# wheretrue/exon-duckdb

Measured on AMD Instinct MI355X. Metric: FASTQ records/sec into DataChunks, higher is better.
Workload: dtype u8; 1 GPU; read_fastq on 10 GB synthetic 150 bp FASTQ (332 B/record, 30120481 records), 1x MI355X, byte-range shards; bytes_per_gpu=9999999692, columns=name,description,sequence,quality_scores as duckdb::string_t + validity

## Files before the change

### exon_duckdb_amd/arrow.py

```python
import ctypes as C

from ._lib import ExgError, load_library
from . import abi


class ReaderResult(C.Structure):
    _fields_ = [("error", C.c_void_p)]


_bound = False


def _lib():
    global _bound
    l = load_library()
    if not _bound:
        l.new_reader.restype = ReaderResult
        l.new_reader.argtypes = [C.c_void_p, C.c_char_p, C.c_size_t, C.c_char_p, C.c_char_p, C.c_char_p]
        _bound = True
    return l


def new_reader(uri, file_format, batch_size=abi.EXG_VECTOR_SIZE, compression=None, filters=None):
    import pyarrow as pa

    l = _lib()
    stream = (C.c_uint64 * 8)()
    enc = lambda s: None if s is None else s.encode()
    res = l.new_reader(C.addressof(stream), enc(uri), batch_size, enc(compression), enc(file_format), enc(filters))
    if res.error:
        msg = C.string_at(res.error).decode("utf-8", "replace")
        C.CDLL(None).free(C.c_void_p(res.error))
        raise ExgError(abi.EXG_E_INVALID_ARG, msg)
    return pa.RecordBatchReader._import_from_c(C.addressof(stream))
```

### exon_duckdb_amd/csrc/exg_fastq_fused.hip

```cpp
#include "exg_fastq.hpp"
#include "exg_fused_core.hpp"

namespace exg {

struct FastqFormat;
static constexpr int kFastqHalves = 3;


__device__ __forceinline__ void fastq_report_utf8(ScanWsHeader *hdr, long long out, int64_t rec_off) {
    atomicMin(&hdr->err_word, ((unsigned long long)out << 8) | EXG_PE_INVALID_UTF8);
    atomicMin(&hdr->err_off, (unsigned long long)rec_off);
}

template <int kMode, class L>
__device__ __forceinline__ void fastq_emit_half(const L &s, const FastqDev &a, ScanWsHeader *hdr, const TileCtx &c,
                                          unsigned long long halo_nl, uint32_t dev_mode, uint32_t lane,
                                          uint32_t wave, unsigned long long *__restrict__ tile_qend,
                                          uint64_t tile_index) {
    const unsigned long long P0 = a.first_line_index - halo_nl;
    const uint32_t i0 = (uint32_t)((3 - P0) & 3);
    const uint32_t i_first = (uint32_t)((3 - (P0 + c.P)) & 3);
    const unsigned long long q_before = c.P > i0 ? (c.P - i0 + 3) / 4 : 0;
    const unsigned long long n_hc = halo_nl > i0 ? (halo_nl - i0 + 3) / 4 : 0;
    const uint32_t n_rec = c.n_lines > i_first ? (c.n_lines - i_first + 3) / 4 : 0;
    const uint64_t ptr_of_e0 = a.payload_base + c.tile_off - kWin;

    if (threadIdx.x == 0 && (c.pass_base == 0 || n_rec)) {
        long long e = 0;
        if (n_rec) {
            e = (long long)c.tile_off + (int)s.nlist[4 + i_first + 4 * (n_rec - 1)] - kWin + 1;
            if ((unsigned long long)e > a.n_bytes) e = (long long)a.n_bytes;
        }
        if (c.pass_base) e |= (long long)(tile_qend[tile_index] & kFarBit);
        if constexpr (kMode != kLean) if (n_rec && s.nlist[i_first] == kNoneE) {
            const long long out0 = (long long)q_before - (long long)n_hc;
            const int e4 = s.nlist[4 + i_first];
            if ((uint64_t)((int64_t)c.tile_off + e4 - kWin) >= a.lead && out0 >= 0 &&
                ((a.flags & EXG_F_NO_STORE) || (unsigned long long)out0 < a.capacity)) {
                FarRec f;
#pragma unroll
                for (int k = 0; k < 5; k++) {
                    const uint32_t idx = i_first + k;
                    f.pos[k] = idx >= 4 ? c.half * kTile + (int32_t)s.nlist[idx] - kWin : s.prev32[idx];
                }
                f.flags = c.is_eof_tile ? 1u : 0u;
                f.out = out0;
                far_rec_of(tile_qend, a.n_bytes)[tile_index] = f;
                hdr->any_far = 1u;
                e |= (long long)kFarBit;
            }
        }
        tile_qend[tile_index] = (unsigned long long)e;
    }
    if (dev_mode >= 3) return;
    const bool no_store = (a.flags & EXG_F_NO_STORE) != 0;

    for (uint32_t jb = 0; jb < n_rec; jb += 64) {
        const uint32_t j = jb + lane;
        const long long out = (long long)(q_before + j) - (long long)n_hc;
        bool act = j < n_rec;
        int i = 0;
        if (act) {
            i = (int)(i_first + 4 * j);
            int e4 = s.nlist[4 + i];
            act = (uint64_t)((int64_t)c.tile_off + e4 - kWin) >= a.lead && out >= 0;
            if (act && !no_store && (unsigned long long)out >= a.capacity) {
                if (wave == 0) atomicOr(&hdr->flags, EXG_RF_CAPACITY);
                act = false;
            }
        }
        bool desc_valid = false;
        if (act) {
            const uint32_t q0 = s.nlist[i];
            uint4 val = make_uint4(0, 0, 0, 0);
            if (q0 == kNoneE) {
                if constexpr (kMode == kLean) {
                    if (wave == 0) {
                        tile_redo_of(tile_qend, a.n_bytes)[opaque_s((uint32_t)(tile_index / kFastqHalves))] = kRedoFar;
                        hdr->any_redo = 1u;
                    }
                }
            } else if (wave <= 1) {
                int s0 = (int)q0 + 1, e0 = s.nlist[i + 1];
                bool name_ok = s0 < e0 && ldb(s, s0) == '@';
                if (e0 > s0 && !(c.is_eof_tile && e0 == c.lim_e) && ldb(s, e0 - 1) == '\r') e0--;
                int ns = s0 + 1 < e0 ? s0 + 1 : e0;
                int sp = e0;
                for (uint32_t aa = (uint32_t)ns & ~3u; aa < (uint32_t)e0 && sp == e0; aa += 32) {
                    uint32_t w8[8];
#pragma unroll
                    for (int q = 0; q < 8; q++) w8[q] = ldw(s, aa + 4 * q);
                    uint32_t bits = 0;
#pragma unroll
                    for (int q = 0; q < 8; q++) bits |= nib4(match4(w8[q], 0x20202020u)) << (4 * q);
                    if (aa < (uint32_t)ns) bits &= 0xFFFFFFFFu << ((uint32_t)ns - aa);
                    if (bits) {
                        uint32_t pos = aa + (uint32_t)__ffs(bits) - 1;
                        if (pos < (uint32_t)e0) sp = (int)pos;
                        break;
                    }
                }
                int ds = sp < e0 ? sp + 1 : e0;
// ... 198 lines not shown
    r.flags = hdr->flags | (hdr->any_redo ? EXG_RF_REDO : 0u);
    r.payload_bytes = 0;
    r.redo_tiles = hdr->n_redo;
    r.error_code = 0;
    r.error_offset = ~0ull;
    r.error_record = ~0ull;
    uint64_t n_rec = (n_owned < a.capacity || (a.flags & EXG_F_NO_STORE)) ? n_owned : a.capacity;
    if (err != kNoError) {
        uint64_t rec = err >> 8;
        r.error_code = (uint32_t)(err & 0xFF);
        r.error_record = rec;
        r.error_offset = err_off;
        if (rec < n_rec) {
            n_rec = rec;
            consumed = err_off > a.lead ? err_off : a.lead;
        }
    }
    r.n_records = n_rec;
    r.consumed_bytes = n_rec ? consumed : a.lead;
    *res = r;
}

int run_fastq_fused(const exg_fastq_scan_args *args, const FastqDev &dev_in, uint8_t *ws, const FastqWsLayout &l,
                    hipStream_t stream, bool full) {
    FastqDev dev = dev_in;
#ifdef EXG_DEV_PROBE
    if (const char *e = getenv("EXG_FASTQ_DEV_MODE")) dev.flags |= ((uint32_t)atoi(e) & 31u) << 8;
#endif
    ScanWsHeader *hdr = reinterpret_cast<ScanWsHeader *>(ws);
    constexpr uint64_t kSuperBytes = (uint64_t)FastqFormat::kHalves * kTile;
    constexpr uint32_t kHalvesHost = FastqFormat::kHalves;
    uint64_t n_super64 = (dev.n_bytes + kSuperBytes - 1) / kSuperBytes;
    if (n_super64 == 0) n_super64 = 1;
    if (n_super64 > 0x7FFFFFF0ull) {
        set_error("exg_fastq_scan: buffer too large for one launch (%llu super-tiles)", (unsigned long long)n_super64);
        return EXG_E_INVALID_ARG;
    }
    uint32_t n_super = (uint32_t)n_super64;
    const uint64_t n = l.n_tiles_fused;
    unsigned int *tileA = reinterpret_cast<unsigned int *>(ws + l.off_tile_desc);
    unsigned long long *tileP = reinterpret_cast<unsigned long long *>(ws + l.off_tile_desc) + n;
    unsigned long long *tile_qend = tileP + 2 * n;
    int32_t *tileL = reinterpret_cast<int32_t *>(ws + l.off_tile_last4);
    FarRec *far_rec = reinterpret_cast<FarRec *>(ws + l.off_far);
    hipLaunchKernelGGL(k_init_hdr, dim3(1), dim3(1), 0, stream, hdr, l.lines_cap, 0u);
    EXG_HIP_CHECK(hipMemsetAsync(tileA, 0, (size_t)n * 24, stream));
    if (dev.lead) {
        int rc = exg_count_newlines(dev.d_in, 0, dev.lead, (uint64_t *)&hdr->halo_nl, stream);
        if (rc) return rc;
    }
    if (full) {
        hipLaunchKernelGGL((k_fused<FastqFormat, kFullPrimary>), dim3(n_super + 1), dim3(kThreads), 0, stream, dev, tileA, tileP, tile_qend, hdr, n_super);
    } else {
        hipLaunchKernelGGL((k_fused<FastqFormat, kLean>), dim3(n_super + 1), dim3(kThreads), 0, stream, dev, tileA, tileP, tile_qend, hdr, n_super);
        hipLaunchKernelGGL((k_fused<FastqFormat, kFullRedo>), dim3(n_super < 1280 ? n_super : 1280), dim3(kThreads), 0, stream, dev, tileA, tileP,
                           tile_qend, hdr, n_super);
    }
    {
        const uint32_t n_halves = n_super * kHalvesHost;
        const uint32_t grid = (n_halves + 255) / 256 < 4096 ? (n_halves + 255) / 256 : 4096;
        hipLaunchKernelGGL(k_fastq_far, dim3(grid), dim3(256), 0, stream, dev, tileA, tileL, tile_qend, far_rec, hdr, n_halves);
    }
    hipLaunchKernelGGL(k_fastq_finalize_fused, dim3(1), dim3(256), 0, stream, dev, hdr, tile_qend, n_super * kHalvesHost,
                       args->d_result);
    EXG_HIP_CHECK(hipGetLastError());
    return EXG_OK;
}

}
```

### exon_duckdb_amd/csrc/exg_fused_core.hpp

```cpp
#pragma once
#include "exg_fastq_ws.hpp"

#ifndef EXG_FIRST_POLL_SLEEP
#define EXG_FIRST_POLL_SLEEP 0
#endif
#ifndef EXG_POLL_SLEEP
#define EXG_POLL_SLEEP 2
#endif

namespace exg {


static constexpr int kTile = kFusedTileBytes;
static constexpr int kMaxHalves = 4;
static constexpr int kWin = kFusedWindow;
static constexpr int kThreads = 256;
static constexpr int kRows = kTile / (kThreads * 16);
static constexpr int kLdsBytes = kWin + kTile + 96;
static constexpr uint32_t kNoneE = 0xFFFFu;

static constexpr uint32_t kFlagA = 1u << 31;
static constexpr uint32_t kNonAsciiA = 1u << 30;
static constexpr uint32_t kCountA = kNonAsciiA - 1;
static constexpr unsigned long long kFlag = 1ull << 63;
// ... 80 lines not shown
            return false;
        }
    }
    return true;
}
__device__ inline bool tiles_non_ascii(const unsigned int *__restrict__ tileA, uint64_t super_bytes, int64_t lo, int64_t hi) {
    if (lo < 0) lo = 0;
    if (hi < lo) return false;
    for (uint64_t t = (uint64_t)lo / super_bytes, t1 = (uint64_t)hi / super_bytes; t <= t1; t++)
        if (tileA[t] & kNonAsciiA) return true;
    return false;
}

__device__ unsigned long long help_count_bytes(const uint8_t *__restrict__ d_in, uint64_t n_bytes, uint64_t b,
                                               uint64_t e, uint32_t lane) {
    unsigned long long cnt = 0;
    if (e > n_bytes) e = n_bytes;
    for (uint64_t off = b + (uint64_t)lane * 16; off < e; off += 1024) {
        uint4 q = *reinterpret_cast<const uint4 *>(d_in + off);
        uint32_t mm = match16(q, 0x0A0A0A0Au);
        if (off + 16 > e) mm &= (1u << (uint32_t)(e - off)) - 1u;
        cnt += __popc(mm);
    }
    for (int o = 32; o > 0; o >>= 1) cnt += __shfl_down(cnt, o, 64);
    return __shfl(cnt, 0, 64);
}

__device__ __forceinline__ uint32_t opaque(uint32_t x) {
    asm volatile("" : "+v"(x));
    return x;
}
__device__ __forceinline__ uint32_t opaque_s(uint32_t x) {
    asm volatile("" : "+s"(x));
    return x;
}
__device__ __forceinline__ uint64_t opaque_s64(uint64_t x) {
    asm volatile("" : "+s"(x));
    return x;
}
template <bool kOn> __device__ __forceinline__ uint32_t opaque_if(uint32_t x) { return kOn ? opaque(x) : x; }
template <bool kOn> __device__ __forceinline__ uint32_t opaque_s_if(uint32_t x) { return kOn ? opaque_s(x) : x; }
template <bool kOn> __device__ __forceinline__ uint64_t opaque_s64_if(uint64_t x) { return kOn ? opaque_s64(x) : x; }
__device__ __forceinline__ unsigned long long rfl64(unsigned long long x) {
    uint32_t lo = __builtin_amdgcn_readfirstlane((uint32_t)x), hi = __builtin_amdgcn_readfirstlane((uint32_t)(x >> 32));
    return ((unsigned long long)hi << 32) | lo;
}
__device__ __forceinline__ unsigned long long ld_desc(const unsigned long long *p) {
    return __hip_atomic_load(p, __ATOMIC_RELAXED, __HIP_MEMORY_SCOPE_AGENT);
}
__device__ __forceinline__ void st_desc(unsigned long long *p, unsigned long long v) {
    __hip_atomic_store(p, v, __ATOMIC_RELAXED, __HIP_MEMORY_SCOPE_AGENT);
}

static constexpr int kScanBatches = 8;

template <int kSuper>
__device__ void scanner_wave(const uint8_t *__restrict__ d_in, uint64_t n_bytes,
                             const unsigned int *__restrict__ tileA, unsigned long long *__restrict__ tileP,
                             uint32_t n_super, uint32_t lane) {
    __builtin_amdgcn_s_setprio(3);
    uint64_t next = 0;
    unsigned long long running = 0;
    unsigned long long t_last = __builtin_amdgcn_s_memrealtime();
    while (next < n_super) {
        unsigned int d[kScanBatches];
#pragma unroll
        for (int k = 0; k < kScanBatches; k++) {
            uint64_t idx = next + (uint64_t)k * 64 + lane;
            d[k] = idx < n_super ? __hip_atomic_load(&tileA[idx], __ATOMIC_RELAXED, __HIP_MEMORY_SCOPE_AGENT) : 0u;
        }
        bool progressed = false;
#pragma unroll
        for (int k = 0; k < kScanBatches; k++) {
            unsigned long long rdy = __ballot((d[k] & kFlagA) != 0);
            int r = rdy == ~0ull ? 64 : __ffsll((long long)~rdy) - 1;
            if (r > 0) {
                uint32_t c = (int)lane < r ? (d[k] & kCountA) : 0u;
                uint32_t inc = wave_incl_sum(c);
                if ((int)lane < r) st_desc(&tileP[next + lane], kFlag | (running + inc - c));
                running += __shfl(inc, 63, 64);
                next += (uint64_t)r;
                progressed = true;
            }
            if (r < 64) break;
        }
        if (progressed) {
            t_last = __builtin_amdgcn_s_memrealtime();
        } else if (__builtin_amdgcn_s_memrealtime() - t_last > 4000) {
            unsigned long long c = help_count_bytes(d_in, n_bytes, next * kSuper, (next + 1) * kSuper, lane);
            if (lane == 0) st_desc(&tileP[next], kFlag | running);
            running += c;
            next++;
            t_last = __builtin_amdgcn_s_memrealtime();
        } else {
            __builtin_amdgcn_s_sleep(1);
        }
    }
}

template <int kSuper>
__device__ unsigned long long wait_prefix(const uint8_t *__restrict__ d_in, uint64_t n_bytes,
                                          unsigned int *__restrict__ tileA,
                                          unsigned long long *__restrict__ tileP, uint32_t st, uint32_t lane, uint32_t &polls) {
    if (st == 0) return 0;
    const unsigned long long t0 = __builtin_amdgcn_s_memrealtime();
    __builtin_amdgcn_s_sleep(EXG_FIRST_POLL_SLEEP);
    for (;;) {
        unsigned long long x = lane == 0 ? ld_desc(&tileP[st]) : 0ull;
        x = (unsigned long long)__shfl((long long)x, 0, 64);
        polls++;
        if (x & kFlag) return x & kVal;
        if (__builtin_amdgcn_s_memrealtime() - t0 > 200000) break;
        __builtin_amdgcn_s_sleep(EXG_POLL_SLEEP);
    }
    unsigned long long sum = 0;
    for (uint64_t b = 0; b < st; b += 64) {
        uint64_t idx = b + lane;
        unsigned long long x = kFlag;
        if (idx < st) {
            unsigned int a32 = __hip_atomic_load(&tileA[idx], __ATOMIC_RELAXED, __HIP_MEMORY_SCOPE_AGENT);
            x = (a32 & kFlagA) ? (kFlag | (a32 & kCountA)) : 0ull;
        }
        unsigned long long miss = __ballot((x & kFlag) == 0);
        while (miss) {
            int l = __ffsll((long long)miss) - 1;
            miss &= miss - 1;
            unsigned long long c = help_count_bytes(d_in, n_bytes, (b + l) * kSuper, (b + l + 1) * kSuper, lane);
            if ((int)lane == l) x = kFlag | c;
        }
        unsigned long long v = idx < st ? (x & kVal) : 0;
        for (int o = 32; o > 0; o >>= 1) v += __shfl_down(v, o, 64);
        sum += __shfl(v, 0, 64);
    }
    return sum;
}

template <int N>
__device__ inline bool far_positions(const FarRec &f, uint32_t st, uint64_t super_bytes, const unsigned int *__restrict__ tileA,
                                     const int32_t *__restrict__ tileL, bool bof, int64_t *p) {
    int need = 0;
#pragma unroll
    for (int k = 0; k < N; k++)
        if (f.pos[k] < 0 && -f.pos[k] > need) need = -f.pos[k];
    int64_t back0 = 0, back1 = 0, back2 = 0, back3 = 0;
    int found = 0;
    for (uint32_t t = st; found < need && t > 0;) {
        t--;
        uint32_t c = tileA[t] & kCountA;
        if (!c) continue;
        if (c > 4) c = 4;
        const int4 l = *reinterpret_cast<const int4 *>(tileL + (uint64_t)t * 4);
        const int64_t base = (int64_t)((uint64_t)t * super_bytes);
        const int32_t e[4] = {l.w, l.z, l.y, l.x};
#pragma unroll
        for (int q = 0; q < 4; q++) {
            if ((uint32_t)q < c && found < need) {
                const int64_t v = base + e[q];
                if (found == 0) back0 = v;
                else if (found == 1) back1 = v;
                else if (found == 2) back2 = v;
                else back3 = v;
                found++;
            }
        }
    }
    if (found < need && bof) {
        const int64_t v = -1;
        if (found == 0) back0 = v;
        else if (found == 1) back1 = v;
        else if (found == 2) back2 = v;
        else back3 = v;
        found++;
    }
    if (found < need) return false;
    const int64_t super_off = (int64_t)((uint64_t)st * super_bytes);
#pragma unroll
    for (int k = 0; k < N; k++) {
        const int32_t c = f.pos[k];
        p[k] = c >= 0 ? super_off + c : c == -1 ? back0 : c == -2 ? back1 : c == -3 ? back2 : back3;
    }
    return true;
}

struct TileCtx {
    uint64_t tile_off;
    unsigned long long P;
    uint32_t n_lines;
    int lim_e;
    bool is_eof_tile;
    bool first_of_buffer;
    bool non_ascii;
    uint32_t pass_base;
    int half;
};

enum { kLean = 0, kFullPrimary = 1, kFullRedo = 2, kFullIndex = 3 };
static constexpr unsigned int kRedoFar = 1u, kRedoDense = 2u, kRedoLast4 = 4u, kRedoUtf8 = 8u;

template <bool kBarriers = true>
__device__ __forceinline__ unsigned int *tile_redo_of(unsigned long long *tile_qend, uint64_t n_bytes) {
    return reinterpret_cast<unsigned int *>(tile_qend - fused_n_tiles(opaque_s64_if<kBarriers>(n_bytes)));
}
template <bool kBarriers = true>
__device__ __forceinline__ int32_t *tile_last4_of(unsigned long long *tile_qend, uint64_t n_bytes) {
    return reinterpret_cast<int32_t *>(tile_qend + fused_n_tiles(opaque_s64_if<kBarriers>(n_bytes)));
}
template <bool kBarriers = true>
__device__ __forceinline__ FarRec *far_rec_of(unsigned long long *tile_qend, uint64_t n_bytes) {
    return reinterpret_cast<FarRec *>(tile_qend + 3 * fused_n_tiles(opaque_s64_if<kBarriers>(n_bytes)));
}

template <class F, int kMode>
__global__ __launch_bounds__(kThreads, kMode == kLean ? F::kMinWavesPerSimd : (kMode == kFullPrimary || kMode == kFullIndex) ? F::kMinWavesPerSimdFull : F::kMinWavesPerSimdRedo) void k_fused(
    typename F::Dev a, unsigned int *__restrict__ tileA, unsigned long long *__restrict__ tileP, unsigned long long *__restrict__ tile_qend,
    ScanWsHeader *hdr, uint32_t n_super) {
    constexpr int kHalves = (kMode == kFullPrimary || kMode == kFullIndex) ? F::kHalvesFull : F::kHalves;
    using FusedLds = FusedLdsT<F::kNlCap, kHalves, (kMode == kLean ? F::kTabMapLean : F::kTabMapFull)>;
    constexpr int kNlCap = F::kNlCap;
    constexpr int kSuper = kTile * kHalves;
    constexpr bool kFull = kMode != kLean;
    constexpr bool kB = F::kBarriers;
    __shared__ __attribute__((aligned(16))) FusedLds s;
    const uint32_t tid = threadIdx.x;
    const uint32_t lane = tid & 63, wave = tid >> 6;
#ifdef EXG_DEV_PROBE
    const uint32_t dev_mode = (a.flags >> 8) & 15u;
#else
    constexpr uint32_t dev_mode = 0;
#endif
    uint32_t st;
    if constexpr (kMode == kFullRedo) {
        if (!hdr->any_redo) return;
        st = blockIdx.x;
    } else {
        if (blockIdx.x == 0) {
            if (wave == 0 && !(dev_mode >= 1 && dev_mode <= 3)) scanner_wave<kHalves * kTile>(a.d_in, a.n_bytes, tileA, tileP, n_super, lane);
            return;
        }
        st = blockIdx.x - 1;
    }
    uint32_t n_redone = 0;
    for (; kMode != kFullRedo || st < n_super; st += gridDim.x) {
    if constexpr (kMode == kFullRedo) {
        if (!tile_redo_of<kB>(tile_qend, a.n_bytes)[st]) continue;
        __syncthreads();
        n_redone++;
    }
    const uint64_t super_off = (uint64_t)st * kSuper;
    const uint8_t *__restrict__ d_in = a.d_in;
    const int64_t lim64 = (int64_t)a.n_bytes - (int64_t)super_off;
    const int lim_s = lim64 < kSuper ? (int)lim64 : kSuper;
    const bool last_super = st + 1 == n_super;

    uint4 v[kHalves * kRows];
    if (lim_s > 0) {
        const uint8_t *base = d_in + super_off;
        const uint32_t last = (((uint32_t)lim_s + 15u) & ~15u) - 16u;
#pragma unroll
        for (int j = 0; j < kHalves * kRows; j++) {
            const uint32_t rel = (uint32_t)(j * kThreads + tid) * 16;
            v[j] = ld_stream16(base + (rel < last ? rel : last));
        }
    } else {
#pragma unroll
        for (int j = 0; j < kHalves * kRows; j++) v[j] = make_uint4(0, 0, 0, 0);
    }
    uint4 wv = make_uint4(0, 0, 0, 0);
    const int64_t woff = (int64_t)super_off - kWin + (int64_t)lane * 16;
    if (wave == 3 && woff >= 0) wv = *reinterpret_cast<const uint4 *>(d_in + woff);

    uint32_t hi = 0, cnt = 0;
#pragma unroll
    for (int j = 0; j < kHalves * kRows; j++) {
        if (lim_s != kSuper && lim_s - (int)(j * kThreads + tid) * 16 <= 0) v[j] = make_uint4(0, 0, 0, 0);
        uint32_t mj = match16(v[j], 0x0A0A0A0Au);
        hi |= v[j].x | v[j].y | v[j].z | v[j].w;
        if (lim_s != kSuper) {
            int rem = lim_s - (int)(j * kThreads + tid) * 16;
            if (rem < 16) mj &= rem <= 0 ? 0u : ((1u << rem) - 1u);
        }
        s.bitmap[j / kRows][(j % kRows) * kThreads + tid] = (uint16_t)mj;
        if constexpr (FusedLds::kHasTabs) s.tabmap[j / kRows][(j % kRows) * kThreads + tid] = (uint16_t)match16(v[j], 0x09090909u);
        cnt += __popc(mj);
    }
    hi &= 0x80808080u;
    for (int o = 32; o > 0; o >>= 1) cnt += __shfl_down(cnt, o, 64);
    if (wave == 3) hi |= (wv.x | wv.y | wv.z | wv.w) & 0x80808080u;
    uint32_t any_hi = __any(hi != 0);
    if (lane == 0) {
        s.hi_or[wave] = any_hi;
        s.wcnt[wave] = cnt;
    }
    __syncthreads();
    const uint32_t n_nl_super = __builtin_amdgcn_readfirstlane(s.wcnt[0] + s.wcnt[1] + s.wcnt[2] + s.wcnt[3]);
    unsigned long long nl_before_half = 0;
    const bool non_ascii = (s.hi_or[0] | s.hi_or[1] | s.hi_or[2] | s.hi_or[3]) != 0;

    const bool analytic = dev_mode >= 1 && dev_mode <= 3;
    if constexpr (kMode != kFullRedo) {
        if (tid == 0 && !analytic)
            __hip_atomic_store(&tileA[st], kFlagA | n_nl_super | (non_ascii ? kNonAsciiA : 0u), __ATOMIC_RELAXED, __HIP_MEMORY_SCOPE_AGENT);
    }
#ifdef EXG_DEV_PROBE
    const unsigned long long t_pub = __builtin_amdgcn_s_memrealtime();
#endif
    const unsigned long long halo_nl = rfl64(hdr->halo_nl);
    if constexpr (kMode != kFullRedo) {
        if (non_ascii && tid == 0) {
            atomicOr(&hdr->flags, EXG_RF_NON_ASCII);
            if constexpr (kMode == kLean) {
                tile_redo_of<kB>(tile_qend, a.n_bytes)[opaque_s_if<kB>(st)] = kRedoUtf8;
                hdr->any_redo = 1u;
            }
        }
    }

#pragma unroll
    for (int h = 0; h < kHalves; h++) {
        const int lim_h = lim_s - h * kTile;
        if (h > 0 && lim_h <= 0) {
            if (tid == 0)
                for (int hh = h; hh < kHalves; hh++) tile_qend[(uint64_t)st * kHalves + hh] = 0;
            break;
        }
        if (h == 0) {
            if (wave == 3) {
                *reinterpret_cast<uint4 *>(s.bytes + lane * 16) = wv;
                if (lane < 4) s.nlist[lane] = (uint16_t)kNoneE;
                if constexpr (kFull) {
                    if (lane < 4) s.prev32[lane] = (int32_t)lane - 4;
                }
                uint32_t wm = woff >= 0 ? match16(wv, 0x0A0A0A0Au) : 0u;
                uint32_t wc = __popc(wm);
                uint32_t wincl = wave_incl_sum(wc);
                uint32_t W = __shfl(wincl, 63, 64);
                uint32_t r = wincl - wc;
                while (wm) {
                    uint32_t b = __ffs(wm) - 1;
                    wm &= wm - 1;
                    int slot = 4 - (int)(W - r);
                    if (slot >= 0) s.nlist[slot] = (uint16_t)(lane * 16 + b);
                    r++;
                }
                if (st == 0 && (a.flags & EXG_F_BOF) && lane == 0) s.nlist[3] = (uint16_t)(kWin - 1);
            }
        } else {
            uint4 t = make_uint4(0, 0, 0, 0);
            if (wave == 3) t = *reinterpret_cast<const uint4 *>(s.bytes + kTile + lane * 16);
            __syncthreads();
            if (wave == 3) {
                *reinterpret_cast<uint4 *>(s.bytes + lane * 16) = t;
                if constexpr (kFull) {
                    if (lane < 4) {
                        const int32_t code = s.carry32[lane], rel = code - (h * kTile - kWin);
                        s.prev32[lane] = code;
                        s.nlist[lane] = (code >= 0 && rel >= 0) ? (uint16_t)rel : (uint16_t)kNoneE;
                    }
                } else {
                    if (lane < 4) s.nlist[lane] = s.carry[lane];
                }
            }
        }
#pragma unroll
        for (int j = 0; j < kRows; j++)
            *reinterpret_cast<uint4 *>(s.bytes + kWin + (j * kThreads + tid) * 16) = v[h * kRows + j];
        uint32_t n_nl_h = 0;
        {
            unsigned long long mask = *reinterpret_cast<const unsigned long long *>(&s.bitmap[h][tid * 4]);
            uint32_t c = (uint32_t)__popcll(mask);
            uint32_t inc = wave_incl_sum(c);
            if (lane == 63) s.wtot[wave] = inc;
            __syncthreads();
            uint32_t r = inc - c + (wave > 0 ? s.wtot[0] : 0) + (wave > 1 ? s.wtot[1] : 0) + (wave > 2 ? s.wtot[2] : 0);
            n_nl_h = __builtin_amdgcn_readfirstlane(s.wtot[0] + s.wtot[1] + s.wtot[2] + s.wtot[3]);
            const uint32_t e0 = kWin + tid * 64;
            while (mask) {
                uint32_t b = (uint32_t)__ffsll((long long)mask) - 1;
                mask &= mask - 1;
                if (r < (uint32_t)kNlCap) s.nlist[4 + r] = (uint16_t)(e0 + b);
                r++;
            }
        }
        if (h == 0) {
            if (wave == 0) {
                unsigned long long pre;
                if constexpr (kMode == kFullRedo) {
                    pre = st ? ld_desc(&tileP[st]) & kVal : 0ull;
                } else if (analytic) {
                    pre = F::analytic_prefix(super_off);
                } else {
                    uint32_t polls = 0;
#ifdef EXG_DEV_PROBE
                    const unsigned long long t_in = __builtin_amdgcn_s_memrealtime();
#endif
                    pre = wait_prefix<kSuper>(d_in, a.n_bytes, tileA, tileP, st, lane, polls);
#ifdef EXG_DEV_PROBE
                    if (kMode == kLean && ((a.flags >> 12) & 1u) && lane == 0) {
                        const unsigned long long now = __builtin_amdgcn_s_memrealtime();
                        FarRec f = {};
                        f.pos[0] = (int32_t)(now - t_in);
                        f.pos[1] = (int32_t)(now - t_pub);
                        f.pos[2] = (int32_t)polls;
                        far_rec_of<kB>(tile_qend, a.n_bytes)[(uint64_t)st * kHalves] = f;
                    }
#endif
                }
                if (lane == 0) s.prefix = pre;
            }
        }
        __syncthreads();

        TileCtx c;
        c.tile_off = super_off + (uint64_t)h * kTile;
        c.P = rfl64(s.prefix) + nl_before_half;
        nl_before_half += n_nl_h;
        c.first_of_buffer = st == 0 && h == 0;
        c.pass_base = 0;
        c.half = h;
        c.non_ascii = non_ascii;
        const bool ends_here = last_super && lim_h <= kTile;
        c.is_eof_tile = ends_here && (a.flags & EXG_F_EOF);
        c.lim_e = (lim_h < kTile ? lim_h : kTile) + kWin;
        uint32_t n_lines = n_nl_h;
        if (c.is_eof_tile) {
            const unsigned long long P0 = a.first_line_index - halo_nl;
            bool unterminated = a.n_bytes > 0 && ldb(s, c.lim_e - 1) != '\n';
            uint32_t n0 = n_lines;
            if (unterminated) n_lines++;
            n_lines += F::eof_extra_lines(P0 + c.P + n_lines);
            if (tid == 0)
                for (uint32_t q = n0; q < n_lines && q < (uint32_t)kNlCap; q++) s.nlist[4 + q] = (uint16_t)c.lim_e;
            __syncthreads();
        }
        c.n_lines = n_lines;
        if (ends_here && tid == 0) {
            hdr->total_nl = c.P + n_nl_h;
            hdr->total_lines = c.P + n_lines;
        }
        const uint64_t half_index = (uint64_t)st * kHalves + h;
        if constexpr (!kFull) {
            if (n_lines > (uint32_t)kNlCap) {
                if (tid == 0) {
                    tile_redo_of<kB>(tile_qend, a.n_bytes)[opaque_s_if<kB>(st)] = kRedoDense;
                    hdr->any_redo = 1u;
                }
                return;
            }
            if (h + 1 < kHalves && tid < 4) {
                uint32_t e = s.nlist[n_lines + tid];
                s.carry[tid] = (e != kNoneE && e >= (uint32_t)kTile) ? (uint16_t)(e - kTile) : (uint16_t)kNoneE;
            }
            if (h + 1 == kHalves || lim_s <= (h + 1) * kTile) {
                if (wave == 0) {
                    const uint32_t k = opaque_if<kB>(lane), idx = n_lines + k;
                    const uint32_t st_here = opaque_s_if<kB>(st);
                    int32_t code = -1;
                    if (k < 4) {
                        const uint32_t e = s.nlist[idx];
                        code = e != kNoneE ? h * kTile + (int32_t)e - kWin : -1;
                        tile_last4_of<kB>(tile_qend, a.n_bytes)[(uint64_t)st_here * 4 + k] = code;
                    }
                    const uint32_t need = n_nl_super < 4u ? n_nl_super : 4u;
                    if (__ballot(k < 4 && k >= 4 - need && code < 0) != 0 && k == 0) {
                        tile_redo_of<kB>(tile_qend, a.n_bytes)[st_here] = kRedoLast4;
                        hdr->any_redo = 1u;
                    }
                }
            }
            F::template emit_half<kLean>(s, a, hdr, c, halo_nl, dev_mode, lane, wave, tile_qend, half_index);
        } else {
            auto fill_list = [&](uint32_t base) {
                unsigned long long mask = *reinterpret_cast<const unsigned long long *>(&s.bitmap[h][tid * 4]);
                uint32_t cc = (uint32_t)__popcll(mask);
                uint32_t inc = wave_incl_sum(cc);
                uint32_t r = inc - cc + (wave > 0 ? s.wtot[0] : 0) + (wave > 1 ? s.wtot[1] : 0) + (wave > 2 ? s.wtot[2] : 0) - base;
                const uint32_t e0 = kWin + tid * 64;
                while (mask) {
                    uint32_t b = (uint32_t)__ffsll((long long)mask) - 1;
                    mask &= mask - 1;
                    if (r < (uint32_t)kNlCap) s.nlist[4 + r] = (uint16_t)(e0 + b);
                    r++;
                }
                if (tid == 0)
                    for (uint32_t q = n_nl_h > base ? n_nl_h : base; q < n_lines && q < base + (uint32_t)kNlCap; q++)
                        s.nlist[4 + q - base] = (uint16_t)c.lim_e;
            };
            const unsigned long long P_half = c.P;
#pragma unroll 1
            for (uint32_t base = 0;;) {
                const uint32_t m = n_lines - base < (uint32_t)kNlCap ? n_lines - base : (uint32_t)kNlCap;
                c.P = P_half + base;
                c.pass_base = base;
                c.n_lines = m;
                if (base + m >= n_lines && tid < 4) {
                    const uint32_t idx = m + tid;
                    const int32_t code = idx >= 4 ? h * kTile + (int32_t)s.nlist[idx] - kWin : s.prev32[idx];
                    s.carry32[tid] = code;
                    if (h + 1 == kHalves || lim_s <= (h + 1) * kTile) tile_last4_of<kB>(tile_qend, a.n_bytes)[(uint64_t)st * 4 + tid] = code;
                }
                F::template emit_half<(kMode == kFullIndex ? kFullIndex : kFullPrimary)>(s, a, hdr, c, halo_nl, dev_mode, lane, wave, tile_qend, half_index);
                base += m;
                if (base >= n_lines) break;
                uint16_t keep = 0;
                if (tid < 4) keep = s.nlist[m + tid];
                __syncthreads();
                if (tid < 4) {
                    s.nlist[tid] = keep;
                    s.prev32[tid] = h * kTile + (int32_t)keep - kWin;
                }
                fill_list(base);
                __syncthreads();
            }
        }
        if (h + 1 < kHalves) __syncthreads();
    }
    if constexpr (kMode != kFullRedo) break;
    }
    if constexpr (kMode == kFullRedo) {
        if (tid == 0 && n_redone) atomicAdd(&hdr->n_redo, n_redone);
    }
}


}
```

### exon_duckdb_amd/csrc/exg_vcf.hip

```cpp
#include <stdlib.h>

#include "exg_fused_core.hpp"
#include "exg_lines.hpp"

#include "exg_parse.hpp"
#include "exg_float_slow.hpp"

namespace exg {

struct VcfDev {
    const uint8_t *d_in;
    uint64_t n_bytes;
    uint64_t lead;
    uint64_t first_line_index;
    uint64_t payload_base;
    uint32_t flags;
    uint32_t pad;
    exg_string_t *d_fields[9];
    int64_t *d_pos;
    float *d_qual;
    uint64_t *d_qual_valid;
    uint64_t *d_formats_valid;
    uint64_t capacity;
    SlowLiteral *d_slow;
// ... 242 lines not shown
        unsigned long long qend_word = 0;
        if (t_rot == 0 && (c.pass_base == 0 || c.n_lines)) {
            long long e = 0;
            if (c.n_lines) {
                e = (long long)c.tile_off + (int)s.nlist[4 + c.n_lines - 1] - kWin + 1;
                if ((unsigned long long)e > a.n_bytes) e = (long long)a.n_bytes;
            }
            if (c.pass_base) e |= (long long)(tile_qend[tile_index] & kFarBit);
            qend_word = (unsigned long long)e;
            tile_qend[tile_index] = qend_word;
        }
        if (dev_mode == 3 || dev_mode == 4) return;
        if constexpr (kMode == kFullIndex) {
            for (uint32_t jb = 0; jb < c.n_lines; jb += kThreads) {
                const uint32_t j = jb + t_rot;
                if (j >= c.n_lines) break;
                const unsigned long long row = c.P + j;
                if (row < a.nl_cap) a.d_nl_pos[row] = (unsigned long long)((long long)c.tile_off + (int)s.nlist[4 + j] - kWin);
                else hdr->overflow = 1u;
            }
            return;
        }
        const bool no_store = (a.flags & EXG_F_NO_STORE) != 0;
        const LdsSrc<L> src{s, a.payload_base + c.tile_off - kWin, s.tabmap[L::kHasTabs ? c.half : 0]};
        for (uint32_t jb = 0; jb < c.n_lines; jb += kThreads) {
            const uint32_t j = jb + t_rot;
            const long long out = (long long)(c.P + j) - (long long)halo_nl;
            bool act = j < c.n_lines;
            int e1 = 0;
            if (act) {
                e1 = s.nlist[4 + j];
                act = (uint64_t)((int64_t)c.tile_off + e1 - kWin) >= a.lead && out >= 0;
                if (act && !no_store && (unsigned long long)out >= a.capacity) {
                    atomicOr(&hdr->flags, EXG_RF_CAPACITY);
                    act = false;
                }
            }
            bool qv = false, rv = false;
            if (act) {
                const uint32_t q0 = s.nlist[3 + j];
                if (q0 == kNoneE) {
                    if constexpr (kMode == kLean) {
                        tile_redo_of<false>(tile_qend, a.n_bytes)[(uint32_t)(tile_index / kVcfHalves)] = kRedoFar;
                        hdr->any_redo = 1u;
                    } else {
                        FarRec f;
                        f.pos[0] = s.prev32[3];
                        f.pos[1] = c.half * kTile + e1 - kWin;
                        f.pos[2] = f.pos[3] = f.pos[4] = 0;
                        f.flags = c.is_eof_tile ? 1u : 0u;
                        f.out = out;
                        far_rec_of<false>(tile_qend, a.n_bytes)[tile_index] = f;
                        hdr->any_far = 1u;
                        tile_qend[tile_index] = qend_word | kFarBit;
                    }
                } else {
                    int s0 = (int)q0 + 1;
                    if (e1 > s0 && !(c.is_eof_tile && e1 == c.lim_e) && ldb(s, e1 - 1) == '\r') e1--;
#ifdef EXG_DEV_PROBE
                    if (dev_mode == 6) continue;
#endif
                    VcfRowInfo r = vcf_line(src, s0, e1, a, (unsigned long long)out, !no_store && dev_mode != 2 && dev_mode != 5);
                    if constexpr (kMode != kLean) {
                        if (!r.code && c.non_ascii && !utf8_valid_lds(s, s0, e1)) r.code = EXG_PE_INVALID_UTF8;
                    }
                    if (r.code) vcf_report(hdr, r.code, (unsigned long long)out, c.tile_off + s0 - kWin);
                    else if (r.slow_len) vcf_slow_qual(hdr, a, c.tile_off + r.slow_s - kWin, (uint32_t)r.slow_len, (unsigned long long)out, c.tile_off + s0 - kWin);
                    qv = r.qual_valid;
                    rv = r.rest_valid;
                }
            }
            if (!no_store) {
                long long out_base = (long long)(c.P + jb + ((wave - rot_w) & 3u) * 64) - (long long)halo_nl;
                unsigned long long qb = __ballot(qv), rb = __ballot(rv);
                store_validity64(a.d_qual_valid, qb, out_base, lane);
                store_validity64(a.d_formats_valid, rb, out_base, lane);
            }
        }
    }
};

struct GlobalSrc {
    const uint8_t *p;
    uint64_t base;
    uint64_t payload_base;
    uint64_t limit;
    __device__ __forceinline__ uint32_t b(int i) const { return p[base + (uint64_t)(int64_t)i]; }
    __device__ __forceinline__ uint32_t u32_slow(uint64_t o) const {
        uint32_t w = 0;
#pragma unroll
        for (int k = 0; k < 4; k++)
            if (o + k < limit) w |= (uint32_t)p[o + k] << (8 * k);
        return w;
    }
    __device__ __forceinline__ uint32_t u32(int i) const {
        const uint64_t o = base + (uint64_t)(int64_t)i, al = o & ~3ull;
        if (al + 8 > limit) return u32_slow(o);
        const uint32_t *q = reinterpret_cast<const uint32_t *>(p + al);
        return __builtin_amdgcn_alignbyte(q[1], q[0], (uint32_t)(o & 3));
    }
    __device__ __forceinline__ void u96(int i, uint32_t *w0, uint32_t *w1, uint32_t *w2) const {
        const uint64_t o = base + (uint64_t)(int64_t)i, al = o & ~3ull;
        if (al + 16 > limit) {
            *w0 = u32_slow(o), *w1 = u32_slow(o + 4), *w2 = u32_slow(o + 8);
            return;
        }
// ... 357 lines not shown
    if (after_fused && !(dev.flags & EXG_F_NO_STORE)) {
        uint64_t words = (dev.capacity + 63) / 64;
        uint32_t g = (uint32_t)((words + 255) / 256 < 1024 ? (words + 255) / 256 : 1024);
        if (words && dev.d_qual_valid)
            hipLaunchKernelGGL(k_clear_words_gated, dim3(g), dim3(256), 0, stream, dev.d_qual_valid, words, gate);
        if (words && dev.d_formats_valid)
            hipLaunchKernelGGL(k_clear_words_gated, dim3(g), dim3(256), 0, stream, dev.d_formats_valid, words, gate);
    }
    int rc = launch_line_index(dev.d_in, dev.n_bytes, dev.lead, ws, l, (dev.flags & EXG_F_EOF) ? 1 : 0, 0, stream, gate);
    if (rc) return rc;
    uint64_t est = dev.n_bytes / 32 + 256;
    uint32_t grid = (uint32_t)((est + 255) / 256 < 2048 ? (est + 255) / 256 : 2048);
    hipLaunchKernelGGL(k_vcf_lines, dim3(grid), dim3(256), 0, stream, dev, nl_pos, hdr, gate);
    hipLaunchKernelGGL(k_vcf_finalize, dim3(1), dim3(256), 0, stream, dev, hdr, (const unsigned long long *)nullptr, 0u,
                       nl_pos, 0, d_result, gate);
    EXG_HIP_CHECK(hipGetLastError());
    return EXG_OK;
}

static int run_vcf_fused(const VcfDev &dev_in, uint8_t *ws, const FastqWsLayout &l, exg_scan_result *d_result,
                         hipStream_t stream, bool full, bool index = false) {
    VcfDev dev = dev_in;
    if (index) {
        dev.d_nl_pos = reinterpret_cast<uint64_t *>(ws + l.off_nl_pos);
        dev.nl_cap = l.lines_cap;
    }
    ScanWsHeader *hdr = reinterpret_cast<ScanWsHeader *>(ws);
    const uint32_t kHalvesHost = full ? VcfFormat::kHalvesFull : VcfFormat::kHalves;
    const uint64_t kSuperBytes = (uint64_t)kHalvesHost * kTile;
    uint64_t n_super64 = (dev.n_bytes + kSuperBytes - 1) / kSuperBytes;
    if (n_super64 == 0) n_super64 = 1;
    if (n_super64 > 0x7FFFFFF0ull) {
        set_error("exg_vcf_scan: buffer too large for one launch");
        return EXG_E_INVALID_ARG;
    }
    uint32_t n_super = (uint32_t)n_super64;
    const uint64_t n = l.n_tiles_fused;
    unsigned int *tileA = reinterpret_cast<unsigned int *>(ws + l.off_tile_desc);
    unsigned long long *tileP = reinterpret_cast<unsigned long long *>(ws + l.off_tile_desc) + n;
    unsigned long long *tile_qend = tileP + 2 * n;
    int32_t *tileL = reinterpret_cast<int32_t *>(ws + l.off_tile_last4);
    FarRec *far_rec = reinterpret_cast<FarRec *>(ws + l.off_far);
    hipLaunchKernelGGL(k_init_hdr, dim3(1), dim3(1), 0, stream, hdr, l.lines_cap, 0u);
    EXG_HIP_CHECK(hipMemsetAsync(tileA, 0, (size_t)n * 24, stream));
    if (dev.lead) {
        int rc = exg_count_newlines(dev.d_in, 0, dev.lead, (uint64_t *)&hdr->halo_nl, stream);
        if (rc) return rc;
    }
    if (index) {
        hipLaunchKernelGGL((k_fused<VcfFormat, kFullIndex>), dim3(n_super + 1), dim3(kThreads), 0, stream, dev, tileA, tileP, tile_qend, hdr, n_super);
    } else if (full) {
        hipLaunchKernelGGL((k_fused<VcfFormat, kFullPrimary>), dim3(n_super + 1), dim3(kThreads), 0, stream, dev, tileA, tileP, tile_qend, hdr, n_super);
    } else {
        hipLaunchKernelGGL((k_fused<VcfFormat, kLean>), dim3(n_super + 1), dim3(kThreads), 0, stream, dev, tileA, tileP, tile_qend, hdr, n_super);
        hipLaunchKernelGGL((k_fused<VcfFormat, kFullRedo>), dim3(n_super < 1024 ? n_super : 1024), dim3(kThreads), 0, stream, dev, tileA, tileP,
                           tile_qend, hdr, n_super);
    }
    if (index) {
        VcfDev rows = dev;
        rows.d_nl_pos = nullptr;
        const uint64_t est = dev.n_bytes / 256 + 256;
        const uint32_t grid = (uint32_t)((est + 255) / 256 < 4096 ? (est + 255) / 256 : 4096);
        hipLaunchKernelGGL(k_vcf_rows, dim3(grid), dim3(256), 0, stream, rows, (const uint64_t *)dev.d_nl_pos, hdr);
    } else {
        const uint32_t n_halves = n_super * kHalvesHost;
        const uint32_t grid = (n_halves + 255) / 256 < 4096 ? (n_halves + 255) / 256 : 4096;
        if (full)
            hipLaunchKernelGGL(k_vcf_far<VcfFormat::kHalvesFull>, dim3(grid), dim3(256), 0, stream, dev, tileA, tileL, tile_qend, far_rec, hdr, n_halves);
        else
            hipLaunchKernelGGL(k_vcf_far<VcfFormat::kHalves>, dim3(grid), dim3(256), 0, stream, dev, tileA, tileL, tile_qend, far_rec, hdr, n_halves);
    }
    hipLaunchKernelGGL(k_vcf_finalize, dim3(1), dim3(256), 0, stream, dev, hdr, tile_qend, n_super * kHalvesHost,
                       (const uint64_t *)nullptr, 1, d_result, (const unsigned int *)nullptr);
    EXG_HIP_CHECK(hipGetLastError());
    return EXG_OK;
}

}

using namespace exg;

extern "C" int exg_vcf_scan(const exg_vcf_scan_args *a) {
    if (!a || !a->d_result || !a->d_workspace || ((uintptr_t)a->d_workspace & 255) || (a->n_bytes && !a->d_input) ||
        ((uintptr_t)a->d_input & 15) || a->lead > a->n_bytes) {
        set_error("exg_vcf_scan: bad arguments (null pointer, unaligned input or workspace, or lead > n_bytes)");
        return EXG_E_INVALID_ARG;
    }
    if (a->flags & ~EXG_F_ALL) {
        set_error("exg_vcf_scan: unknown flag bits 0x%x", a->flags & ~EXG_F_ALL);
        return EXG_E_INVALID_ARG;
    }
    FastqWsLayout l = fastq_ws_layout(a->n_bytes, a->workspace_bytes);
    if (a->workspace_bytes < fastq_ws_layout(a->n_bytes, 0).off_nl_pos + 64) {
        set_error("exg_vcf_scan: workspace too small");
        return EXG_E_INVALID_ARG;
    }
    VcfDev dev;
    dev.d_in = (const uint8_t *)a->d_input;
    dev.n_bytes = a->n_bytes;
    dev.lead = a->lead;
    dev.first_line_index = 0;
    dev.payload_base = a->payload_base;
    dev.flags = a->flags;
#ifdef EXG_DEV_PROBE
    if (const char *e = getenv("EXG_VCF_DEV_MODE")) dev.flags |= ((uint32_t)atoi(e) & 15u) << 8;
#endif
    dev.pad = 0;
// ... 37 lines not shown
```

Before: 13.84 billion records/s.

## Peel tail superblock from lean pass into redo kernel, drop bounds checks

The lean fused pass now covers only whole superblocks. The final, partial superblock is always processed by the redo kernel, which sets the tail prefix, marks redo needs and publishes descriptors for it. This lets the lean kernel drop the per-load bounds handling and the byte clamp, and use straight 16-byte global loads (optionally nontemporal). The cost is more complex redo logic, with a tail that is serialized after the lean kernel and new correctness risks around redo flags. The Python ctypes binding caching was also removed.

```diff
diff --git a/exon_duckdb_amd/arrow.py b/exon_duckdb_amd/arrow.py
--- a/exon_duckdb_amd/arrow.py
+++ b/exon_duckdb_amd/arrow.py
@@ -8,16 +8,10 @@
     _fields_ = [("error", C.c_void_p)]
 
 
-_bound = False
-
-
 def _lib():
-    global _bound
     l = load_library()
-    if not _bound:
-        l.new_reader.restype = ReaderResult
-        l.new_reader.argtypes = [C.c_void_p, C.c_char_p, C.c_size_t, C.c_char_p, C.c_char_p, C.c_char_p]
-        _bound = True
+    l.new_reader.restype = ReaderResult
+    l.new_reader.argtypes = [C.c_void_p, C.c_char_p, C.c_size_t, C.c_char_p, C.c_char_p, C.c_char_p]
     return l
 
 
diff --git a/exon_duckdb_amd/csrc/exg_fastq_fused.hip b/exon_duckdb_amd/csrc/exg_fastq_fused.hip
--- a/exon_duckdb_amd/csrc/exg_fastq_fused.hip
+++ b/exon_duckdb_amd/csrc/exg_fastq_fused.hip
@@ -29,7 +29,9 @@
         long long e = 0;
         if (n_rec) {
             e = (long long)c.tile_off + (int)s.nlist[4 + i_first + 4 * (n_rec - 1)] - kWin + 1;
-            if ((unsigned long long)e > a.n_bytes) e = (long long)a.n_bytes;
+            if constexpr (kMode != kLean) {
+                if ((unsigned long long)e > a.n_bytes) e = (long long)a.n_bytes;
+            }
         }
         if (c.pass_base) e |= (long long)(tile_qend[tile_index] & kFarBit);
         if constexpr (kMode != kLean) if (n_rec && s.nlist[i_first] == kNoneE) {
@@ -48,6 +50,10 @@
                 far_rec_of(tile_qend, a.n_bytes)[tile_index] = f;
                 hdr->any_far = 1u;
                 e |= (long long)kFarBit;
+                if (c.tail_marks) {
+                    tile_redo_of(tile_qend, a.n_bytes)[(uint32_t)(tile_index / kFastqHalves)] = kRedoFar;
+                    hdr->any_redo = 1u;
+                }
             }
         }
         tile_qend[tile_index] = (unsigned long long)e;
@@ -352,7 +358,8 @@
     if (full) {
         hipLaunchKernelGGL((k_fused<FastqFormat, kFullPrimary>), dim3(n_super + 1), dim3(kThreads), 0, stream, dev, tileA, tileP, tile_qend, hdr, n_super);
     } else {
-        hipLaunchKernelGGL((k_fused<FastqFormat, kLean>), dim3(n_super + 1), dim3(kThreads), 0, stream, dev, tileA, tileP, tile_qend, hdr, n_super);
+        if (n_super > 1)
+            hipLaunchKernelGGL((k_fused<FastqFormat, kLean>), dim3(n_super), dim3(kThreads), 0, stream, dev, tileA, tileP, tile_qend, hdr, n_super);
         hipLaunchKernelGGL((k_fused<FastqFormat, kFullRedo>), dim3(n_super < 1280 ? n_super : 1280), dim3(kThreads), 0, stream, dev, tileA, tileP,
                            tile_qend, hdr, n_super);
     }
diff --git a/exon_duckdb_amd/csrc/exg_fused_core.hpp b/exon_duckdb_amd/csrc/exg_fused_core.hpp
--- a/exon_duckdb_amd/csrc/exg_fused_core.hpp
+++ b/exon_duckdb_amd/csrc/exg_fused_core.hpp
@@ -156,9 +156,19 @@
     __hip_atomic_store(p, v, __ATOMIC_RELAXED, __HIP_MEMORY_SCOPE_AGENT);
 }
 
+__device__ __forceinline__ uint4 ld_stream16_global(uint64_t addr) {
+    typedef const exg_v4u __attribute__((address_space(1))) *gptr;
+#ifdef EXG_NT_LOAD
+    const exg_v4u v = __builtin_nontemporal_load((gptr)addr);
+#else
+    const exg_v4u v = *(gptr)addr;
+#endif
+    return make_uint4(v.x, v.y, v.z, v.w);
+}
+
 static constexpr int kScanBatches = 8;
 
-template <int kSuper>
+template <int kSuper, bool kTailPrefix>
 __device__ void scanner_wave(const uint8_t *__restrict__ d_in, uint64_t n_bytes,
                              const unsigned int *__restrict__ tileA, unsigned long long *__restrict__ tileP,
                              uint32_t n_super, uint32_t lane) {
@@ -199,6 +209,9 @@
         } else {
             __builtin_amdgcn_s_sleep(1);
         }
+    }
+    if constexpr (kTailPrefix) {
+        if (lane == 0) st_desc(&tileP[n_super], kFlag | running);
     }
 }
 
@@ -296,6 +309,7 @@
     bool non_ascii;
     uint32_t pass_base;
     int half;
+    bool tail_marks;
 };
 
 enum { kLean = 0, kFullPrimary = 1, kFullRedo = 2, kFullIndex = 3 };
@@ -332,32 +346,49 @@
 #else
     constexpr uint32_t dev_mode = 0;
 #endif
+    constexpr bool kWhole = kMode == kLean;
     uint32_t st;
     if constexpr (kMode == kFullRedo) {
-        if (!hdr->any_redo) return;
         st = blockIdx.x;
+        if (tid == 0) s.prefix = hdr->any_redo;
+        __syncthreads();
+        if (!s.prefix) {
+            if (st != (n_super - 1) % gridDim.x) return;
+            st = n_super - 1;
+        }
     } else {
         if (blockIdx.x == 0) {
-            if (wave == 0 && !(dev_mode >= 1 && dev_mode <= 3)) scanner_wave<kHalves * kTile>(a.d_in, a.n_bytes, tileA, tileP, n_super, lane);
+            if (wave == 0 && !(dev_mode >= 1 && dev_mode <= 3))
+                scanner_wave<kHalves * kTile, kWhole>(a.d_in, a.n_bytes, tileA, tileP, kWhole ? n_super - 1 : n_super, lane);
             return;
         }
         st = blockIdx.x - 1;
     }
     uint32_t n_redone = 0;
     for (; kMode != kFullRedo || st < n_super; st += gridDim.x) {
+    const bool is_tail = kMode == kFullRedo && st + 1 == n_super;
     if constexpr (kMode == kFullRedo) {
-        if (!tile_redo_of<kB>(tile_qend, a.n_bytes)[st]) continue;
+        if (!is_tail) {
+            if (!tile_redo_of<kB>(tile_qend, a.n_bytes)[st]) continue;
+            n_redone++;
+        }
         __syncthreads();
-        n_redone++;
     }
     const uint64_t super_off = (uint64_t)st * kSuper;
     const uint8_t *__restrict__ d_in = a.d_in;
     const int64_t lim64 = (int64_t)a.n_bytes - (int64_t)super_off;
-    const int lim_s = lim64 < kSuper ? (int)lim64 : kSuper;
-    const bool last_super = st + 1 == n_super;
+    const int lim_s = kWhole ? kSuper : lim64 < kSuper ? (int)lim64 : kSuper;
+    const bool last_super = !kWhole && st + 1 == n_super;
 
     uint4 v[kHalves * kRows];
-    if (lim_s > 0) {
+    if constexpr (kWhole) {
+        const uint32_t rel = tid * 16;
+#pragma unroll
+        for (int j = 0; j < kHalves * kRows; j++) {
+            const uint64_t base = opaque_s64((uint64_t)d_in + super_off + (uint64_t)(j * kThreads * 16));
+            v[j] = ld_stream16_global(base + rel);
+        }
+    } else if (lim_s > 0) {
         const uint8_t *base = d_in + super_off;
         const uint32_t last = (((uint32_t)lim_s + 15u) & ~15u) - 16u;
 #pragma unroll
@@ -401,7 +432,7 @@
     const bool non_ascii = (s.hi_or[0] | s.hi_or[1] | s.hi_or[2] | s.hi_or[3]) != 0;
 
     const bool analytic = dev_mode >= 1 && dev_mode <= 3;
-    if constexpr (kMode != kFullRedo) {
+    if (kMode != kFullRedo || is_tail) {
         if (tid == 0 && !analytic)
             __hip_atomic_store(&tileA[st], kFlagA | n_nl_super | (non_ascii ? kNonAsciiA : 0u), __ATOMIC_RELAXED, __HIP_MEMORY_SCOPE_AGENT);
     }
@@ -409,10 +440,10 @@
     const unsigned long long t_pub = __builtin_amdgcn_s_memrealtime();
 #endif
     const unsigned long long halo_nl = rfl64(hdr->halo_nl);
-    if constexpr (kMode != kFullRedo) {
+    if (kMode != kFullRedo || is_tail) {
         if (non_ascii && tid == 0) {
             atomicOr(&hdr->flags, EXG_RF_NON_ASCII);
-            if constexpr (kMode == kLean) {
+            if constexpr (kMode == kLean || kMode == kFullRedo) {
                 tile_redo_of<kB>(tile_qend, a.n_bytes)[opaque_s_if<kB>(st)] = kRedoUtf8;
                 hdr->any_redo = 1u;
             }
@@ -488,10 +519,10 @@
         if (h == 0) {
             if (wave == 0) {
                 unsigned long long pre;
-                if constexpr (kMode == kFullRedo) {
+                if (analytic) {
+                    pre = F::analytic_prefix(super_off);
+                } else if constexpr (kMode == kFullRedo) {
                     pre = st ? ld_desc(&tileP[st]) & kVal : 0ull;
-                } else if (analytic) {
-                    pre = F::analytic_prefix(super_off);
                 } else {
                     uint32_t polls = 0;
 #ifdef EXG_DEV_PROBE
@@ -522,6 +553,7 @@
         c.pass_base = 0;
         c.half = h;
         c.non_ascii = non_ascii;
+        c.tail_marks = is_tail;
         const bool ends_here = last_super && lim_h <= kTile;
         c.is_eof_tile = ends_here && (a.flags & EXG_F_EOF);
         c.lim_e = (lim_h < kTile ? lim_h : kTile) + kWin;
@@ -590,6 +622,10 @@
                         s.nlist[4 + q - base] = (uint16_t)c.lim_e;
             };
             const unsigned long long P_half = c.P;
+            if (is_tail && tid == 0 && n_lines > (uint32_t)kNlCap) {
+                tile_redo_of<kB>(tile_qend, a.n_bytes)[st] = kRedoDense;
+                hdr->any_redo = 1u;
+            }
 #pragma unroll 1
             for (uint32_t base = 0;;) {
                 const uint32_t m = n_lines - base < (uint32_t)kNlCap ? n_lines - base : (uint32_t)kNlCap;
@@ -600,7 +636,14 @@
                     const uint32_t idx = m + tid;
                     const int32_t code = idx >= 4 ? h * kTile + (int32_t)s.nlist[idx] - kWin : s.prev32[idx];
                     s.carry32[tid] = code;
-                    if (h + 1 == kHalves || lim_s <= (h + 1) * kTile) tile_last4_of<kB>(tile_qend, a.n_bytes)[(uint64_t)st * 4 + tid] = code;
+                    if (h + 1 == kHalves || lim_s <= (h + 1) * kTile) {
+                        tile_last4_of<kB>(tile_qend, a.n_bytes)[(uint64_t)st * 4 + tid] = code;
+                        const uint32_t need = n_nl_super < 4u ? n_nl_super : 4u;
+                        if (is_tail && tid >= 4 - need && (code < 0 || code < h * kTile - kWin)) {
+                            tile_redo_of<kB>(tile_qend, a.n_bytes)[st] = kRedoLast4;
+                            hdr->any_redo = 1u;
+                        }
+                    }
                 }
                 F::template emit_half<(kMode == kFullIndex ? kFullIndex : kFullPrimary)>(s, a, hdr, c, halo_nl, dev_mode, lane, wave, tile_qend, half_index);
                 base += m;
@@ -619,6 +662,10 @@
         if (h + 1 < kHalves) __syncthreads();
     }
     if constexpr (kMode != kFullRedo) break;
+    if (is_tail) {
+        __syncthreads();
+        if (tid == 0 && __hip_atomic_load(&tile_redo_of<kB>(tile_qend, a.n_bytes)[st], __ATOMIC_RELAXED, __HIP_MEMORY_SCOPE_AGENT)) n_redone++;
+    }
     }
     if constexpr (kMode == kFullRedo) {
         if (tid == 0 && n_redone) atomicAdd(&hdr->n_redo, n_redone);
diff --git a/exon_duckdb_amd/csrc/exg_vcf.hip b/exon_duckdb_amd/csrc/exg_vcf.hip
--- a/exon_duckdb_amd/csrc/exg_vcf.hip
+++ b/exon_duckdb_amd/csrc/exg_vcf.hip
@@ -318,6 +318,10 @@
                         f.out = out;
                         far_rec_of<false>(tile_qend, a.n_bytes)[tile_index] = f;
                         hdr->any_far = 1u;
+                        if (c.tail_marks) {
+                            tile_redo_of<false>(tile_qend, a.n_bytes)[(uint32_t)(tile_index / kVcfHalves)] = kRedoFar;
+                            hdr->any_redo = 1u;
+                        }
                         tile_qend[tile_index] = qend_word | kFarBit;
                     }
                 } else {
@@ -781,7 +785,8 @@
     } else if (full) {
         hipLaunchKernelGGL((k_fused<VcfFormat, kFullPrimary>), dim3(n_super + 1), dim3(kThreads), 0, stream, dev, tileA, tileP, tile_qend, hdr, n_super);
     } else {
-        hipLaunchKernelGGL((k_fused<VcfFormat, kLean>), dim3(n_super + 1), dim3(kThreads), 0, stream, dev, tileA, tileP, tile_qend, hdr, n_super);
+        if (n_super > 1)
+            hipLaunchKernelGGL((k_fused<VcfFormat, kLean>), dim3(n_super), dim3(kThreads), 0, stream, dev, tileA, tileP, tile_qend, hdr, n_super);
         hipLaunchKernelGGL((k_fused<VcfFormat, kFullRedo>), dim3(n_super < 1024 ? n_super : 1024), dim3(kThreads), 0, stream, dev, tileA, tileP,
                            tile_qend, hdr, n_super);
     }
```

Result: no change. 13.96 billion records/s, median of 6 (+0.8%).
